# cmbant/getdist

Hardware: AMD Instinct MI355X
Metric: 2D KDE densities/sec (triangle, 50 params, 1e+07 samples) (higher is better)
Workload: dtype f64

## Files before the change

### getdist_amd/csrc/binning.hip

```cpp
#include "ctx.hpp"

#include <array>
#include <map>

#define LDS_HIST_BYTES (128 * 1024)

struct BinDiv {
    double binmin, width, rcp;
};
__device__ __forceinline__ BinDiv make_bindiv(double binmin, double width) {
    BinDiv d;
    d.binmin = binmin, d.width = width;
    const unsigned long long mant = (unsigned long long)__double_as_longlong(width) & 0xFFFFFFFFFFFFFull;
    d.rcp = (mant == 0xFFFFFFFFFFFFFull) ? 0.0 : 1.0 / width;
    return d;
}
__device__ __forceinline__ double bin_quotient(double x, const BinDiv& d) {
    const double n = x - d.binmin;
    double q = n * d.rcp;
    double r = fma(-q, d.width, n);
    q = fma(r, d.rcp, q);
    r = fma(-q, d.width, n);
    q = fma(r, d.rcp, q);
    if (!(fabs(q) < 1e300) || d.rcp == 0.0) q = n / d.width;
// ... 201 lines not shown
            const uint4 ax = gload_u4(P.ix + i);
            const uint4 ay = gload_u4(P.iy + i);
            double2 wv[4];
#pragma unroll
            for (int q = 0; q < 4; ++q)
                wv[q] = HAS_W ? *reinterpret_cast<const double2*>(w + i + 2 * q) : make_double2(1.0, 1.0);
            const unsigned xs[4] = {ax.x, ax.y, ax.z, ax.w}, ys[4] = {ay.x, ay.y, ay.z, ay.w};
#pragma unroll
            for (int q = 0; q < 4; ++q) {
#pragma unroll
                for (int h = 0; h < 2; ++h) {
                    const unsigned cx = (xs[q] >> (16 * h)) & 0xFFFFu, cy = (ys[q] >> (16 * h)) & 0xFFFFu;
                    const unsigned r = cy - (unsigned)row0;
                    if (r < (unsigned)R && cx < (unsigned)F && cy < (unsigned)F)
                        lds_add<BinT>(&sh[r * F + cx], h ? wv[q].y : wv[q].x);
                }
            }
        }
        if (threadIdx.x == 0)
            for (int64_t i = hi8; i < hi; ++i) {
                const unsigned cx = P.ix[i], cy = P.iy[i];
                const unsigned r = cy - (unsigned)row0;
                if (r < (unsigned)R && cx < (unsigned)F && cy < (unsigned)F)
                    lds_add<BinT>(&sh[r * F + cx], HAS_W ? w[i] : 1.0);
            }
    } else {
        const int64_t hi2 = lo + ((hi - lo) & ~(int64_t)1);
        for (int64_t i = lo + 2 * (int64_t)threadIdx.x; i < hi2; i += 2 * (int64_t)blockDim.x) {
            const double2 xv = gload_d2(P.x + i);
            const double2 yv = gload_d2(P.y + i);
            double2 wv = make_double2(1.0, 1.0);
            if (HAS_W) wv = *reinterpret_cast<const double2*>(w + i);
            int cx0, cy0, cx1, cy1;
            if (MODE == 0) {
                cx0 = bin_round(xv.x, bdx), cy0 = bin_round(yv.x, bdy);
                cx1 = bin_round(xv.y, bdx), cy1 = bin_round(yv.y, bdy);
            } else {
                cx0 = bin_trunc(xv.x, bdx), cx1 = bin_trunc(xv.y, bdx);
                const double p0 = P.r0 * xv.x + P.r1 * yv.x, p1 = P.r0 * xv.y + P.r1 * yv.y;
                cy0 = bin_trunc(p0, bdy), cy1 = bin_trunc(p1, bdy);
            }
            unsigned r = (unsigned)cy0 - (unsigned)row0;
            if (r < (unsigned)R && (unsigned)cx0 < (unsigned)F && (unsigned)cy0 < (unsigned)F)
                lds_add<BinT>(&sh[r * F + cx0], wv.x);
            r = (unsigned)cy1 - (unsigned)row0;
            if (r < (unsigned)R && (unsigned)cx1 < (unsigned)F && (unsigned)cy1 < (unsigned)F)
                lds_add<BinT>(&sh[r * F + cx1], wv.y);
        }
        if (threadIdx.x == 0 && hi2 < hi) {
            const double xv = P.x[hi2], yv = P.y[hi2];
            int cx, cy;
            if (MODE == 0) {
                cx = bin_round(xv, bdx), cy = bin_round(yv, bdy);
            } else {
                cx = bin_trunc(xv, bdx);
                cy = bin_trunc(P.r0 * xv + P.r1 * yv, bdy);
            }
            const unsigned r = (unsigned)cy - (unsigned)row0;
            if (r < (unsigned)R && (unsigned)cx < (unsigned)F && (unsigned)cy < (unsigned)F)
                lds_add<BinT>(&sh[r * F + cx], HAS_W ? w[hi2] : 1.0);
        }
    }
    __syncthreads();
    flush_stripe<BinT>(sh, row0, R, F, hist_all + (int64_t)pair * F * F, nchunks == 1);
}


template <bool HAS_W8>
__global__ void __launch_bounds__(1024) k_hist2d_u16(const Hist2DPair* __restrict__ pairs, int B, int64_t N, int F,
                                                     int R, int nstripes, const unsigned char* __restrict__ w8,
                                                     double* __restrict__ hist_all, int* __restrict__ overflow) {
    extern __shared__ double sh_raw[];
    unsigned int* sh = reinterpret_cast<unsigned int*>(sh_raw);
    __shared__ double red[16];
    int pair, chunk, stripe;
    decode_block(nstripes, 1, pair, chunk, stripe);
    if (pair >= B) return;
    const Hist2DPair P = pairs[pair];
    const BinDiv bdx = make_bindiv(P.bx, P.wx), bdy = make_bindiv(P.by, P.wy);
    const int row0 = stripe * R;
    const int nwords = (R * F + 1) / 2;
    for (int i = threadIdx.x; i < nwords; i += blockDim.x) sh[i] = 0;
    __syncthreads();
    unsigned int nacc = 0;
    auto visit = [&](unsigned cx, unsigned cy, unsigned wt) {
        const unsigned r = cy - (unsigned)row0;
        if (r < (unsigned)R && cx < (unsigned)F && cy < (unsigned)F && (!HAS_W8 || wt != 0u)) {
            const unsigned a = r * (unsigned)F + cx;
            atomicAdd(&sh[a >> 1], wt << ((a & 1u) * 16u));
            nacc += wt;
        }
    };
    auto visit8 = [&](const uint4& ax, const uint4& ay, unsigned wlo, unsigned whi) {
        const unsigned xs[4] = {ax.x, ax.y, ax.z, ax.w}, ys[4] = {ay.x, ay.y, ay.z, ay.w};
#pragma unroll
        for (int q = 0; q < 4; ++q) {
            const unsigned ww = (q < 2 ? wlo : whi) >> ((q & 1) * 16);
            visit(xs[q] & 0xFFFFu, ys[q] & 0xFFFFu, HAS_W8 ? (ww & 0xFFu) : 1u);
            visit(xs[q] >> 16, ys[q] >> 16, HAS_W8 ? ((ww >> 8) & 0xFFu) : 1u);
        }
    };
    const int64_t N16 = N & ~(int64_t)15;
    for (int64_t i = 16 * (int64_t)threadIdx.x; i < N16; i += 16 * (int64_t)blockDim.x) {
        const uint4 ax0 = gload_u4(P.ix + i), ay0 = gload_u4(P.iy + i);
        const uint4 ax1 = gload_u4(P.ix + i + 8), ay1 = gload_u4(P.iy + i + 8);
        uint4 wv = make_uint4(0, 0, 0, 0);
        if (HAS_W8) wv = *reinterpret_cast<const uint4*>(w8 + i);
        visit8(ax0, ay0, wv.x, wv.y);
        visit8(ax1, ay1, wv.z, wv.w);
    }
    if (threadIdx.x == 0)
        for (int64_t i = N16; i < N; ++i) visit(P.ix[i], P.iy[i], HAS_W8 ? (unsigned)w8[i] : 1u);
    __syncthreads();
    double* hist = hist_all + (int64_t)pair * F * F;
    unsigned int total = 0;
    for (int i = threadIdx.x; i < R * F; i += blockDim.x) {
        const int r = row0 + i / F;
        if (r >= F) break;
        const unsigned int v = (sh[i >> 1] >> ((i & 1) * 16)) & 0xFFFFu;
        total += v;
        hist[(int64_t)r * F + (i % F)] = (double)v;
    }
    const double t = block_sum((double)total, red), a = block_sum((double)nacc, red);
    if (threadIdx.x == 0 && t != a) atomicOr(&overflow[pair], 1);
}

struct Hist2DPair8 {
    const unsigned char* ix;
    const unsigned char* iy;
};

template <int DEPTH>
__global__ void __launch_bounds__(1024) k_hist2d_u8_pf(const Hist2DPair8* __restrict__ pairs, int B, int64_t N,
                                                       double* __restrict__ hist_all, int* __restrict__ overflow, int nchunks = 1,
                                                       unsigned int* __restrict__ part = nullptr) {
    extern __shared__ double sh_raw[];
    unsigned int* sh = reinterpret_cast<unsigned int*>(sh_raw);
    double* red = sh_raw + 16384;
    const int units = B * nchunks, per_xcd = (units + 7) / 8;
    const int unit = (blockIdx.x & 7) * per_xcd + (blockIdx.x >> 3);
    if (unit >= units || (int)(blockIdx.x >> 3) >= per_xcd) return;
    const int pair = unit / nchunks, chunk = unit - pair * nchunks;
    const Hist2DPair8 P = pairs[pair];
    const int64_t nvec_all = N >> 4;
    int64_t per = (nvec_all + nchunks - 1) / nchunks;
    per = (per + 1023) & ~(int64_t)1023;
    const int64_t v0 = min(nvec_all, (int64_t)chunk * per), v1 = (nchunks == 1) ? nvec_all : min(nvec_all, v0 + per);
    const bool last = chunk == nchunks - 1;
    const uint4* gx = reinterpret_cast<const uint4*>(P.ix) + v0;
    const uint4* gy = reinterpret_cast<const uint4*>(P.iy) + v0;
    for (int i = threadIdx.x; i < 32768; i += 1024) sh[i] = 0;
    __syncthreads();
    auto visit2 = [&](unsigned v) {
        atomicAdd(&sh[v & 0x7fffu], __builtin_amdgcn_ubfe(v, 15, 1) * 0xffffu + 1u);
        atomicAdd(&sh[__builtin_amdgcn_ubfe(v, 16, 15)], (v >> 31) * 0xffffu + 1u);
    };
    auto visit16 = [&](const uint4& ax, const uint4& ay) {
        const unsigned xs[4] = {ax.x, ax.y, ax.z, ax.w}, ys[4] = {ay.x, ay.y, ay.z, ay.w};
#pragma unroll
        for (int q = 0; q < 4; ++q) {
            visit2(__builtin_amdgcn_perm(ys[q], xs[q], 0x05010400u));
            visit2(__builtin_amdgcn_perm(ys[q], xs[q], 0x07030602u));
        }
    };
    const int64_t nvec = v1 - v0;
    const int64_t K = (nvec >> 10) / DEPTH * DEPTH;
    if (K > 0) {
        uint4 rx[DEPTH], ry[DEPTH];
#pragma unroll
        for (int d = 0; d < DEPTH; ++d) {
            rx[d] = gload_u4(gx + d * 1024 + threadIdx.x), ry[d] = gload_u4(gy + d * 1024 + threadIdx.x);
            __builtin_amdgcn_sched_barrier(0);
        }
        for (int64_t k = 0; k < K; k += DEPTH) {
            const int64_t kn = (k + DEPTH < K ? k + DEPTH : K - DEPTH) * 1024 + threadIdx.x;
#pragma unroll
            for (int d = 0; d < DEPTH; ++d) {
                visit16(rx[d], ry[d]);
                rx[d] = gload_u4(gx + kn + d * 1024), ry[d] = gload_u4(gy + kn + d * 1024);
                __builtin_amdgcn_sched_barrier(0);
            }
        }
    }
    for (int64_t u = K * 1024 + threadIdx.x; u < nvec; u += 1024) visit16(gload_u4(gx + u), gload_u4(gy + u));
    if (threadIdx.x == 0 && last)
        for (int64_t i = nvec_all << 4; i < N; ++i) {
            const unsigned a = ((unsigned)P.iy[i] << 8) | (unsigned)P.ix[i];
            atomicAdd(&sh[a & 0x7fffu], (a >> 15) * 0xffffu + 1u);
        }
    __syncthreads();
    if (nchunks > 1) {
        unsigned int* out = part + (int64_t)unit * 32768;
        unsigned int total = 0;
        for (int i = 4 * threadIdx.x; i < 32768; i += 4096) {
            const uint4 c = *reinterpret_cast<const uint4*>(&sh[i]);
            total += (c.x & 0xffffu) + (c.x >> 16) + (c.y & 0xffffu) + (c.y >> 16) + (c.z & 0xffffu) + (c.z >> 16) + (c.w & 0xffffu) + (c.w >> 16);
            *reinterpret_cast<uint4*>(&out[i]) = c;
        }
        const double t = block_sum((double)total, red);
        const double mine = (double)((v1 - v0) << 4) + (last ? (double)(N - (nvec_all << 4)) : 0.0);
        if (threadIdx.x == 0 && t != mine) atomicOr(&overflow[pair], 1);
        return;
    }
    double* hist = hist_all + (int64_t)pair * 65536;
    unsigned int total = 0;
    for (int i = 2 * threadIdx.x; i < 32768; i += 2048) {
        const uint2 c = *reinterpret_cast<const uint2*>(&sh[i]);
        total += (c.x & 0xffffu) + (c.x >> 16) + (c.y & 0xffffu) + (c.y >> 16);
        *reinterpret_cast<double2*>(&hist[i]) = make_double2((double)(c.x & 0xffffu), (double)(c.y & 0xffffu));
        *reinterpret_cast<double2*>(&hist[i + 32768]) = make_double2((double)(c.x >> 16), (double)(c.y >> 16));
    }
    const double t = block_sum((double)total, red);
    if (threadIdx.x == 0 && t != (double)N) atomicOr(&overflow[pair], 1);
}

__global__ void __launch_bounds__(256) k_p8_reduce(const unsigned int* __restrict__ part, int nchunks, double* __restrict__ hist_all) {
    const int pair = blockIdx.y;
    const int i = (blockIdx.x * 256 + threadIdx.x) * 4;
    const unsigned int* p = part + (int64_t)pair * nchunks * 32768 + i;
    unsigned int lo[4] = {0, 0, 0, 0}, hi[4] = {0, 0, 0, 0};
    for (int c = 0; c < nchunks; ++c) {
        const uint4 v = *reinterpret_cast<const uint4*>(p + (int64_t)c * 32768);
        lo[0] += v.x & 0xffffu, hi[0] += v.x >> 16, lo[1] += v.y & 0xffffu, hi[1] += v.y >> 16;
        lo[2] += v.z & 0xffffu, hi[2] += v.z >> 16, lo[3] += v.w & 0xffffu, hi[3] += v.w >> 16;
    }
    double* hist = hist_all + (int64_t)pair * 65536;
    *reinterpret_cast<double2*>(&hist[i]) = make_double2((double)lo[0], (double)lo[1]);
    *reinterpret_cast<double2*>(&hist[i + 2]) = make_double2((double)lo[2], (double)lo[3]);
    *reinterpret_cast<double2*>(&hist[i + 32768]) = make_double2((double)hi[0], (double)hi[1]);
    *reinterpret_cast<double2*>(&hist[i + 32768 + 2]) = make_double2((double)hi[2], (double)hi[3]);
}

static int pick_chunks(const gd_ctx* ctx, int64_t units, int64_t rows);
static int u8_chunks(const gd_ctx* ctx, int B, int64_t N) {
    if (B >= 2 * ctx->cu_count) return 1;
    return pick_chunks(ctx, B, N);
}

struct PrebinCol8 {
    const double* x;
    unsigned char* idx;
    double binmin, width;
};

__global__ void __launch_bounds__(256) k_prebin8_batch(const PrebinCol8* __restrict__ colsv, int64_t N, int F,
                                                       unsigned long long* __restrict__ bad) {
    const PrebinCol8 C = colsv[blockIdx.y];
    const BinDiv bd = make_bindiv(C.binmin, C.width);
    const int64_t gtid = (int64_t)blockIdx.x * 256 + threadIdx.x, gsz = (int64_t)gridDim.x * 256;
    const int64_t N8 = N & ~(int64_t)7;
    unsigned nbad = 0;
    for (int64_t i = 8 * gtid; i < N8; i += 8 * gsz) {
        double2 v[4];
#pragma unroll
        for (int q = 0; q < 4; ++q) v[q] = gload_d2(C.x + i + 2 * q);
        unsigned o[8];
#pragma unroll
        for (int q = 0; q < 4; ++q) {
            const int a = bin_round(v[q].x, bd), b = bin_round(v[q].y, bd);
            nbad += ((unsigned)a >= (unsigned)F) + ((unsigned)b >= (unsigned)F);
            o[2 * q] = (unsigned)a & 0xffu;
            o[2 * q + 1] = (unsigned)b & 0xffu;
        }
        uint2 pk;
        pk.x = o[0] | (o[1] << 8) | (o[2] << 16) | (o[3] << 24);
        pk.y = o[4] | (o[5] << 8) | (o[6] << 16) | (o[7] << 24);
        *reinterpret_cast<uint2*>(C.idx + i) = pk;
    }
    if (gtid == 0)
        for (int64_t i = N8; i < N; ++i) {
            const int a = bin_round(C.x[i], bd);
            nbad += ((unsigned)a >= (unsigned)F);
            C.idx[i] = (unsigned char)a;
        }
    if (nbad) atomicAdd(&bad[blockIdx.y], (unsigned long long)nbad);
}

struct PrebinColB {
    const double* x;
    const unsigned short* bq;
    void* idx;
    double binmin, width;
    double mn, inv_scale, slack;
    int nb, pad;
};

__global__ void __launch_bounds__(256) k_bucket_lut(const PrebinColB* __restrict__ colsv, int F, int nbmax,
                                                    unsigned short* __restrict__ lut) {
    const PrebinColB C = colsv[blockIdx.y];
    const int b = blockIdx.x * 256 + threadIdx.x;
    if (b >= C.nb) return;
    unsigned short v = 0xFFFF;
    if (b > 0 && b < C.nb - 1) {
        const BinDiv bd = make_bindiv(C.binmin, C.width);
        const double x_lo = (C.mn + ((double)b - 1e-3) * C.inv_scale) - C.slack;
        const double x_hi = (C.mn + ((double)b + 1.0 + 1e-3) * C.inv_scale) + C.slack;
        const int a = bin_round(x_lo, bd), c = bin_round(x_hi, bd);
        if (a == c && (unsigned)a < (unsigned)F) v = (unsigned short)a;
    }
    lut[(int64_t)blockIdx.y * nbmax + b] = v;
}

template <bool OUT8>
__global__ void __launch_bounds__(512) k_prebin_bq(const PrebinColB* __restrict__ colsv, int64_t N, int64_t R, int cap, int nbmax,
                                                   const unsigned short* __restrict__ lut, unsigned int* __restrict__ lists,
                                                   int* __restrict__ counts) {
    extern __shared__ unsigned short slut[];
    __shared__ int nlist;
    const PrebinColB C = colsv[blockIdx.y];
    {
        const uint4* src = reinterpret_cast<const uint4*>(lut + (int64_t)blockIdx.y * nbmax);
        uint4* dst = reinterpret_cast<uint4*>(slut);
        for (int i = threadIdx.x; i < C.nb / 8; i += 512) dst[i] = src[i];
    }
    if (threadIdx.x == 0) nlist = 0;
    __syncthreads();
    const int mask = C.nb - 1;
    unsigned int* mylist = lists + ((int64_t)blockIdx.y * gridDim.x + blockIdx.x) * cap;
    const int64_t g_lo = (int64_t)blockIdx.x * R / 8;
    int64_t g_hi = g_lo + R / 8;
    if (g_hi > N / 8) g_hi = N / 8;
    auto group = [&](const uint4& v, int64_t g) {
        const unsigned wd[4] = {v.x, v.y, v.z, v.w};
        unsigned o[8];
#pragma unroll
        for (int e = 0; e < 8; ++e) {
            unsigned r = slut[(wd[e >> 1] >> (16 * (e & 1))) & mask];
            if (r == 0xFFFFu) {
                const int pos = atomicAdd(&nlist, 1);
                if (pos < cap) mylist[pos] = (unsigned)(8 * g + e);
                r = 0;
            }
            o[e] = r;
        }
        if (OUT8) {
            uint2 pk;
            pk.x = o[0] | (o[1] << 8) | (o[2] << 16) | (o[3] << 24);
            pk.y = o[4] | (o[5] << 8) | (o[6] << 16) | (o[7] << 24);
            *reinterpret_cast<uint2*>((unsigned char*)C.idx + 8 * g) = pk;
        } else {
            uint4 pk;
            pk.x = o[0] | (o[1] << 16), pk.y = o[2] | (o[3] << 16), pk.z = o[4] | (o[5] << 16), pk.w = o[6] | (o[7] << 16);
            *reinterpret_cast<uint4*>((unsigned short*)C.idx + 8 * g) = pk;
        }
    };
    constexpr int U = 4;
    int64_t i = g_lo + threadIdx.x;
    for (; i + (U - 1) * 512 < g_hi; i += U * 512) {
        uint4 v[U];
#pragma unroll
        for (int q = 0; q < U; ++q) v[q] = gload_u4(C.bq + 8 * (i + q * 512));
#pragma unroll
        for (int q = 0; q < U; ++q) group(v[q], i + q * 512);
    }
    for (; i < g_hi; i += 512) group(gload_u4(C.bq + 8 * i), i);
    __syncthreads();
    if (threadIdx.x == 0) counts[(int64_t)blockIdx.y * gridDim.x + blockIdx.x] = nlist;
}

template <bool OUT8>
__global__ void __launch_bounds__(256) k_prebin_fix(const PrebinColB* __restrict__ colsv, int64_t N, int64_t R, int cap, int F,
                                                    const unsigned int* __restrict__ lists, const int* __restrict__ counts,
                                                    unsigned long long* __restrict__ bad) {
    const PrebinColB C = colsv[blockIdx.y];
    const BinDiv bd = make_bindiv(C.binmin, C.width);
    unsigned nbad = 0;
    auto settle = [&](int64_t row) {
        const int a = bin_round(C.x[row], bd);
        if (OUT8) {
            nbad += ((unsigned)a >= (unsigned)F);
            ((unsigned char*)C.idx)[row] = (unsigned char)a;
        } else {
            ((unsigned short*)C.idx)[row] = (unsigned)a < (unsigned)F ? (unsigned short)a : (unsigned short)0xFFFF;
        }
    };
    const int cnt = counts[(int64_t)blockIdx.y * gridDim.x + blockIdx.x];
    if (cnt <= cap) {
        const unsigned int* mylist = lists + ((int64_t)blockIdx.y * gridDim.x + blockIdx.x) * cap;
        int k = threadIdx.x;
        for (; k + 3 * 256 < cnt; k += 4 * 256) {
            unsigned int r[4];
#pragma unroll
            for (int q = 0; q < 4; ++q) r[q] = mylist[k + q * 256];
            double xv[4];
#pragma unroll
            for (int q = 0; q < 4; ++q) xv[q] = C.x[r[q]];
#pragma unroll
            for (int q = 0; q < 4; ++q) {
                const int a = bin_round(xv[q], bd);
                if (OUT8) {
                    nbad += ((unsigned)a >= (unsigned)F);
                    ((unsigned char*)C.idx)[r[q]] = (unsigned char)a;
                } else {
                    ((unsigned short*)C.idx)[r[q]] = (unsigned)a < (unsigned)F ? (unsigned short)a : (unsigned short)0xFFFF;
                }
            }
        }
        for (; k < cnt; k += 256) settle((int64_t)mylist[k]);
    } else {
        const int64_t lo = (int64_t)blockIdx.x * R;
        int64_t hi = lo + R;
        if (hi > N / 8 * 8) hi = N / 8 * 8;
        for (int64_t r = lo + threadIdx.x; r < hi; r += 256) settle(r);
    }
    if (blockIdx.x == gridDim.x - 1)
        for (int64_t r = N / 8 * 8 + threadIdx.x; r < N; r += 256) settle(r);
    if (OUT8 && nbad) atomicAdd(&bad[blockIdx.y], (unsigned long long)nbad);
}

struct BucketRoute {
    std::vector<PrebinColB> recs;
    std::vector<int> slot_of;
    int nbmax = 0;
};
static BucketRoute bucket_route(gd_ctx* ctx, const int32_t* cols, int32_t ncols, const double* binmin, const double* width,
                                void* const* d_idx) {
    BucketRoute R;
    R.slot_of.assign((size_t)ncols, -1);
    if (!ctx->bq || getenv("GDHIP_NO_BUCKET_COLS")) return R;
    {
        const char* e = getenv("GDHIP_BUCKET_ROUTE_MIN");
        const int min_cols = e ? atoi(e) : 24;
        if (ncols < min_cols) return R;
    }
    BucketCols& B = *ctx->bq;
    std::lock_guard<std::mutex> g(B.mu);
    if (!B.buf || B.ld != ctx->ld) return R;
    for (int c = 0; c < ncols; ++c) {
        const int col = cols[c];
        if (col < 0 || col >= B.n || B.nb[col] <= 0) continue;
        PrebinColB r;
        memset(&r, 0, sizeof r);
        r.x = ctx->cols + (int64_t)col * ctx->ld;
        r.bq = B.buf + (int64_t)col * B.ld;
        r.idx = d_idx[c];
        r.binmin = binmin[c], r.width = width[c];
        r.mn = B.mn[col];
        r.inv_scale = 1.0 / B.scale[col];
        const double mx = r.mn + (double)B.nb[col] * r.inv_scale;
        r.slack = 8.0 * 2.220446049250313e-16 * fmax(fabs(r.mn), fabs(mx));
        r.nb = B.nb[col];
        if (!(r.inv_scale > 0) || !std::isfinite(r.inv_scale) || !std::isfinite(r.slack)) continue;
        R.slot_of[c] = (int)R.recs.size();
        R.recs.push_back(r);
        if (r.nb > R.nbmax) R.nbmax = r.nb;
    }
    return R;
}
struct BucketShape {
    int nblk;
    int64_t R;
    int cap;
};
static BucketShape bucket_shape(const gd_ctx* ctx, int nc) {
    BucketShape S;
    int nblk = (4 * ctx->cu_count + nc - 1) / nc;
    int64_t R = (ctx->N + nblk - 1) / nblk;
    if (R < 131072) R = 131072;
    R = (R + 4095) / 4096 * 4096;
    nblk = (int)((ctx->N + R - 1) / R);
    if (nblk < 1) nblk = 1;
    S.nblk = nblk, S.R = R, S.cap = (int)(R / 8);
    if (const char* e = getenv("GDHIP_BUCKET_LIST_CAP"))
        if (atoi(e) > 0 && atoi(e) < S.cap) S.cap = atoi(e);
    return S;
}
static int64_t bucket_route_bytes(const gd_ctx* ctx, const BucketRoute& R) {
    if (R.recs.empty()) return 0;
    const int nc = (int)R.recs.size();
    const BucketShape S = bucket_shape(ctx, nc);
    return ((int64_t)nc * sizeof(PrebinColB) + 255) / 256 * 256 + ((int64_t)nc * R.nbmax * 2 + 255) / 256 * 256 +
           ((int64_t)nc * 8 + 255) / 256 * 256 + ((int64_t)nc * S.nblk * 4 + 255) / 256 * 256 + (int64_t)nc * S.nblk * S.cap * 4 + 256;
}
template <bool OUT8>
static int bucket_route_launch(gd_ctx* ctx, const BucketRoute& R, char* base, int F, unsigned long long** bad_dev) {
    const int nc = (int)R.recs.size();
    const BucketShape S = bucket_shape(ctx, nc);
    int64_t off = 0;
    auto take = [&](int64_t bytes) {
        int64_t o = off;
        off += (bytes + 255) / 256 * 256;
        return o;
    };
    const int64_t o_recs = take((int64_t)nc * sizeof(PrebinColB)), o_lut = take((int64_t)nc * R.nbmax * 2), o_bad = take((int64_t)nc * 8),
                  o_cnt = take((int64_t)nc * S.nblk * 4), o_list = take((int64_t)nc * S.nblk * S.cap * 4);
    PrebinColB* d_recs = (PrebinColB*)(base + o_recs);
    unsigned short* d_lut = (unsigned short*)(base + o_lut);
    unsigned long long* d_bad = (unsigned long long*)(base + o_bad);
    int* d_cnt = (int*)(base + o_cnt);
    unsigned int* d_list = (unsigned int*)(base + o_list);
    GD_TRY(gd_h2d(ctx, d_recs, R.recs.data(), (size_t)nc * sizeof(PrebinColB)));
    GD_HIP(hipMemsetAsync(d_bad, 0, (size_t)nc * 8, ctx->stream));
    k_bucket_lut<<<dim3(R.nbmax / 256, nc), 256, 0, ctx->stream>>>(d_recs, F, R.nbmax, d_lut);
    GD_KERNEL_CHECK();
    const size_t lds = (size_t)R.nbmax * 2;
    GD_HIP(hipFuncSetAttribute((const void*)k_prebin_bq<OUT8>, hipFuncAttributeMaxDynamicSharedMemorySize, (int)lds));
    k_prebin_bq<OUT8><<<dim3(S.nblk, nc), 512, lds, ctx->stream>>>(d_recs, ctx->N, S.R, S.cap, R.nbmax, d_lut, d_list, d_cnt);
    GD_KERNEL_CHECK();
    k_prebin_fix<OUT8><<<dim3(S.nblk, nc), 256, 0, ctx->stream>>>(d_recs, ctx->N, S.R, S.cap, F, d_list, d_cnt, d_bad);
    GD_KERNEL_CHECK();
    *bad_dev = d_bad;
    return GD_OK;
}

#ifndef P16_UNROLL
#define P16_UNROLL 4
#endif
template <int MODE>
__global__ void __launch_bounds__(1024) k_hist2d_f64_p16(const Hist2DPair* __restrict__ pairs, int B, int64_t N, int F, int R,
                                                         int nstripes, int nchunks, int tile_major,
                                                         unsigned int* __restrict__ part, int* __restrict__ overflow) {
    extern __shared__ double sh_raw[];
    unsigned int* sh = reinterpret_cast<unsigned int*>(sh_raw);
    __shared__ double red[16];
    int pair, chunk, stripe;
    if (tile_major)
        decode_block_tiles(B, nstripes, nchunks, pair, chunk, stripe);
    else
        decode_block(nstripes, nchunks, pair, chunk, stripe);
    if (pair >= B) return;
    const Hist2DPair P = pairs[pair];
    const BinDiv bdx = make_bindiv(P.bx, P.wx), bdy = make_bindiv(P.by, P.wy);
    const int row0 = stripe * R;
    const int nwords = (R * F + 1) / 2;
    for (int i = threadIdx.x; i < nwords; i += 1024) sh[i] = 0;
    __syncthreads();
    int64_t per = (N + nchunks - 1) / nchunks;
    per = (per + 7) & ~(int64_t)7;
    const int64_t lo = (int64_t)chunk * per;
    int64_t hi = lo + per;
    if (hi > N) hi = N;
    if (hi < lo) hi = lo;
    unsigned int nacc = 0;
    auto visit = [&](double xv, double yv) {
        int cx, cy;
        if (MODE == 0) {
            cx = bin_round(xv, bdx), cy = bin_round(yv, bdy);
        } else {
            cx = bin_trunc(xv, bdx);
            cy = bin_trunc(P.r0 * xv + P.r1 * yv, bdy);
        }
        const unsigned r = (unsigned)cy - (unsigned)row0;
        if (r < (unsigned)R && (unsigned)cx < (unsigned)F && (unsigned)cy < (unsigned)F) {
            const unsigned a = r * (unsigned)F + (unsigned)cx;
            atomicAdd(&sh[a >> 1], 1u << ((a & 1u) * 16u));
            nacc += 1;
        }
    };
    const int64_t hi2 = lo + ((hi - lo) & ~(int64_t)1);
    int64_t i = lo + 2 * (int64_t)threadIdx.x;
    for (; i + (int64_t)(P16_UNROLL - 1) * 2 * 1024 < hi2; i += (int64_t)P16_UNROLL * 2 * 1024) {
        double2 xv[P16_UNROLL], yv[P16_UNROLL];
#pragma unroll
        for (int u = 0; u < P16_UNROLL; ++u) {
            xv[u] = gload_d2(P.x + i + (int64_t)u * 2 * 1024);
            yv[u] = gload_d2(P.y + i + (int64_t)u * 2 * 1024);
        }
#pragma unroll
        for (int u = 0; u < P16_UNROLL; ++u) {
            visit(xv[u].x, yv[u].x);
            visit(xv[u].y, yv[u].y);
        }
    }
    for (; i < hi2; i += 2 * 1024) {
        const double2 xv = gload_d2(P.x + i);
        const double2 yv = gload_d2(P.y + i);
        visit(xv.x, yv.x);
        visit(xv.y, yv.y);
    }
    if (threadIdx.x == 0 && hi2 < hi) visit(P.x[hi2], P.y[hi2]);
    __syncthreads();
    unsigned int* dst = part + (((int64_t)pair * nchunks + chunk) * nstripes + stripe) * (int64_t)nwords;
    unsigned int total = 0;
    for (int i = threadIdx.x; i < nwords; i += 1024) {
        const unsigned int v = sh[i];
        total += (v & 0xffffu) + (v >> 16);
        dst[i] = v;
    }
    const double t = block_sum((double)total, red), a = block_sum((double)nacc, red);
    if (threadIdx.x == 0 && t != a) atomicOr(&overflow[pair], 1);
}

__global__ void __launch_bounds__(1024) k_hist2d_u16_chunks(const Hist2DPair* __restrict__ pairs, int B, int64_t N, int F, int R,
                                                            int nstripes, int nchunks, unsigned int* __restrict__ part,
                                                            int* __restrict__ overflow) {
    extern __shared__ double sh_raw[];
    unsigned int* sh = reinterpret_cast<unsigned int*>(sh_raw);
    __shared__ double red[16];
    int pair, chunk, stripe;
    decode_block(nstripes, nchunks, pair, chunk, stripe);
    if (pair >= B) return;
    const Hist2DPair P = pairs[pair];
    const int row0 = stripe * R;
    const int nwords = (R * F + 1) / 2;
    for (int i = threadIdx.x; i < nwords; i += 1024) sh[i] = 0;
    __syncthreads();
    int64_t per = (N + nchunks - 1) / nchunks;
    per = (per + 7) & ~(int64_t)7;
    const int64_t lo = (int64_t)chunk * per;
    int64_t hi = lo + per;
    if (hi > N) hi = N;
    unsigned int nacc = 0;
    auto visit = [&](unsigned cx, unsigned cy) {
        const unsigned r = cy - (unsigned)row0;
        if (r < (unsigned)R && cx < (unsigned)F && cy < (unsigned)F) {
            const unsigned a = r * (unsigned)F + cx;
            atomicAdd(&sh[a >> 1], 1u << ((a & 1u) * 16u));
            nacc += 1;
        }
    };
    const int64_t hi8 = lo < hi ? lo + ((hi - lo) & ~(int64_t)7) : lo;
    auto visit8 = [&](const uint4& ax, const uint4& ay) {
        const unsigned xs[4] = {ax.x, ax.y, ax.z, ax.w}, ys[4] = {ay.x, ay.y, ay.z, ay.w};
#pragma unroll
        for (int q = 0; q < 4; ++q) {
            visit(xs[q] & 0xFFFFu, ys[q] & 0xFFFFu);
            visit(xs[q] >> 16, ys[q] >> 16);
        }
    };
    constexpr int DEPTH = 3;
    const int64_t nvec = (hi8 - lo) >> 3;
    const int64_t K = (nvec >> 10) / DEPTH * DEPTH;
    const uint4* gx = reinterpret_cast<const uint4*>(P.ix + lo);
    const uint4* gy = reinterpret_cast<const uint4*>(P.iy + lo);
    if (K > 0) {
        uint4 rx[DEPTH], ry[DEPTH];
#pragma unroll
        for (int d = 0; d < DEPTH; ++d) {
            rx[d] = gload_u4(gx + d * 1024 + threadIdx.x), ry[d] = gload_u4(gy + d * 1024 + threadIdx.x);
            __builtin_amdgcn_sched_barrier(0);
        }
        for (int64_t k = 0; k < K; k += DEPTH) {
            const int64_t kn = (k + DEPTH < K ? k + DEPTH : K - DEPTH) * 1024 + threadIdx.x;
#pragma unroll
            for (int d = 0; d < DEPTH; ++d) {
                visit8(rx[d], ry[d]);
                rx[d] = gload_u4(gx + kn + d * 1024), ry[d] = gload_u4(gy + kn + d * 1024);
                __builtin_amdgcn_sched_barrier(0);
            }
        }
    }
    for (int64_t u = K * 1024 + threadIdx.x; u < nvec; u += 1024) visit8(gload_u4(gx + u), gload_u4(gy + u));
    if (threadIdx.x == 0)
        for (int64_t i = hi8; i < hi; ++i) visit(P.ix[i], P.iy[i]);
    __syncthreads();
    unsigned int* dst = part + (((int64_t)pair * nchunks + chunk) * nstripes + stripe) * (int64_t)nwords;
    unsigned int total = 0;
    for (int i = threadIdx.x; i < nwords; i += 1024) {
        const unsigned int v = sh[i];
        total += (v & 0xffffu) + (v >> 16);
        dst[i] = v;
    }
    const double t = block_sum((double)total, red), a = block_sum((double)nacc, red);
    if (threadIdx.x == 0 && t != a) atomicOr(&overflow[pair], 1);
}

__global__ void __launch_bounds__(256) k_p16_reduce(const unsigned int* __restrict__ part, int F, int R, int nstripes, int nchunks,
                                                    double* __restrict__ hist_all) {
    const int pair = blockIdx.z, stripe = blockIdx.y;
    const int nwords = (R * F + 1) / 2;
    const int rows = min(R, F - stripe * R);
    const int wd = blockIdx.x * 256 + threadIdx.x;
    if (2 * wd >= rows * F) return;
    const int64_t step = (int64_t)nstripes * nwords;
    const unsigned int* p = part + ((int64_t)pair * nchunks * nstripes + stripe) * (int64_t)nwords + wd;
    unsigned int lo = 0, hi = 0;
    int c = 0;
    for (; c + 8 <= nchunks; c += 8) {
        unsigned int v[8];
#pragma unroll
        for (int q = 0; q < 8; ++q) v[q] = __builtin_nontemporal_load(p + (c + q) * step);
#pragma unroll
        for (int q = 0; q < 8; ++q) lo += v[q] & 0xffffu, hi += v[q] >> 16;
    }
    for (; c < nchunks; ++c) {
        const unsigned int v = p[c * step];
        lo += v & 0xffffu, hi += v >> 16;
    }
    double* hist = hist_all + (int64_t)pair * F * F + (int64_t)stripe * R * F;
    hist[2 * wd] = (double)lo;
    if (2 * wd + 1 < rows * F) hist[2 * wd + 1] = (double)hi;
}

__global__ void k_minmax_affine(const Hist2DPair* __restrict__ pairs, int64_t N, double* __restrict__ part) {
    __shared__ double red[16];
    const Hist2DPair P = pairs[blockIdx.y];
    double mn = INFINITY, mx = -INFINITY;
    const int64_t gtid = (int64_t)blockIdx.x * blockDim.x + threadIdx.x, gsz = (int64_t)gridDim.x * blockDim.x;
    const int64_t Ne = N & ~(int64_t)1;
    for (int64_t i = 2 * gtid; i < Ne; i += 2 * gsz) {
        const double2 xv = gload_d2(P.x + i);
        const double2 yv = gload_d2(P.y + i);
        const double p0 = P.r0 * xv.x + P.r1 * yv.x, p1 = P.r0 * xv.y + P.r1 * yv.y;
        mn = fmin(mn, fmin(p0, p1));
        mx = fmax(mx, fmax(p0, p1));
    }
    if (gtid == 0 && Ne < N) {
        const double p0 = P.r0 * P.x[Ne] + P.r1 * P.y[Ne];
        mn = fmin(mn, p0);
        mx = fmax(mx, p0);
    }
    const double r0 = block_min(mn, red), r1 = block_max(mx, red);
    if (threadIdx.x == 0) {
        double* p = part + ((int64_t)blockIdx.y * gridDim.x + blockIdx.x) * 2;
        p[0] = r0, p[1] = r1;
    }
}

#define MMG_COLS 8
#define MMG_PAIRS 16
struct MinmaxGroup {
    const double* col[MMG_COLS];
    double r0[MMG_PAIRS], r1[MMG_PAIRS];
    int a[MMG_PAIRS], b[MMG_PAIRS];
    int ncols, npairs;
};

__global__ void __launch_bounds__(256) k_minmax_affine_grouped(const MinmaxGroup* __restrict__ groups, int64_t N,
                                                               double* __restrict__ part) {
    __shared__ double2 slot[MMG_COLS][256];
    __shared__ double red[16];
    const MinmaxGroup& G = groups[blockIdx.y];
    const int ncols = G.ncols, npairs = G.npairs;
    double mn[MMG_PAIRS], mx[MMG_PAIRS];
#pragma unroll
    for (int p = 0; p < MMG_PAIRS; ++p) mn[p] = INFINITY, mx[p] = -INFINITY;
    const int64_t gtid = (int64_t)blockIdx.x * blockDim.x + threadIdx.x, gsz = (int64_t)gridDim.x * blockDim.x;
    const int64_t Ne = N & ~(int64_t)1;
    for (int64_t i = 2 * gtid; i < Ne; i += 2 * gsz) {
        double2 v[MMG_COLS];
#pragma unroll
        for (int c = 0; c < MMG_COLS; ++c) v[c] = gload_d2(G.col[min(c, ncols - 1)] + i);
        __builtin_amdgcn_sched_barrier(0);
#pragma unroll
        for (int c = 0; c < MMG_COLS; ++c) slot[c][threadIdx.x] = v[c];
#pragma unroll
        for (int p = 0; p < MMG_PAIRS; ++p)
            if (p < npairs) {
                const double2 xv = slot[G.a[p]][threadIdx.x], yv = slot[G.b[p]][threadIdx.x];
                const double p0 = G.r0[p] * xv.x + G.r1[p] * yv.x, p1 = G.r0[p] * xv.y + G.r1[p] * yv.y;
                mn[p] = fmin(mn[p], fmin(p0, p1));
                mx[p] = fmax(mx[p], fmax(p0, p1));
            }
    }
    if (gtid == 0 && Ne < N) {
#pragma unroll
        for (int p = 0; p < MMG_PAIRS; ++p)
            if (p < npairs) {
                const double p0 = G.r0[p] * G.col[G.a[p]][Ne] + G.r1[p] * G.col[G.b[p]][Ne];
                mn[p] = fmin(mn[p], p0);
                mx[p] = fmax(mx[p], p0);
            }
    }
    double* out = part + ((int64_t)blockIdx.y * gridDim.x + blockIdx.x) * MMG_PAIRS * 2;
#pragma unroll
    for (int p = 0; p < MMG_PAIRS; ++p)
        if (p < npairs) {
            const double r0 = block_min(mn[p], red), r1 = block_max(mx[p], red);
            if (threadIdx.x == 0) out[2 * p] = r0, out[2 * p + 1] = r1;
        }
}

static int pick_chunks(const gd_ctx* ctx, int64_t units, int64_t rows) {
    int best = 1;
    double best_cost = 1e30;
    for (int c = 1; c <= 16; ++c) {
        if ((int64_t)c * 65536 > rows && c > 1) break;
        const int64_t blocks = units * c;
        const double rounds = (double)((blocks + ctx->cu_count - 1) / ctx->cu_count);
        const double cost = rounds / c + 0.004 * c;
        if (cost < best_cost - 1e-12) best_cost = cost, best = c;
    }
    return best;
}

template <int MODE>
static int launch_hist2d(gd_ctx* ctx, int B, const std::vector<Hist2DPair>& hp, int F, double* d_hist, bool allow_p16 = true);

template <int MODE>
static int launch_hist2d_p16(gd_ctx* ctx, int B, const std::vector<Hist2DPair>& hp, int F, double* d_hist) {
    int R = LDS_HIST_BYTES / (F * 2);
    if (R > F) R = F;
    const int nstripes = (F + R - 1) / R;
    int nchunks = pick_chunks(ctx, (int64_t)B * nstripes, ctx->N);
    const int nwords = (R * F + 1) / 2;
    int tile_major = 0;
    if (B >= 16 && nstripes == 1 && ctx->N >= (1 << 20) && getenv("GDHIP_P16_TILE_MAJOR") != nullptr) {
        int64_t tiles = (ctx->N + 131071) / 131072;
        const int64_t cap = ((int64_t)3 << 30) / ((int64_t)B * nwords * 4);
        if (tiles > cap) tiles = cap;
        if (tiles > nchunks) nchunks = (int)tiles, tile_major = 1;
    }
    const int units = (B * nchunks + 7) / 8 * 8;
    const int64_t nblocks = (int64_t)units * nstripes;
    int64_t off = 0;
    auto take = [&](int64_t bytes) {
        int64_t o = off;
        off += (bytes + 255) / 256 * 256;
        return o;
    };
    const int64_t o_pairs = take((int64_t)B * sizeof(Hist2DPair)), o_flags = take((int64_t)B * 4),
                  o_part = take((int64_t)B * nchunks * nstripes * nwords * 4);
// ... 988 lines not shown
```

Before: 50080.

## Fuse bucket prebin fix-up pass into LUT kernel with batched list appends

Merges the separate fix-up kernel into the LUT prebin kernel, so each block settles its undecided rows right after a block barrier. That removes one kernel launch and the per-block counts array. Undecided samples are now gathered into a per-lane bitmask and appended with one LDS atomicAdd per unrolled iteration instead of one per sample. The load loop is software-pipelined to prefetch the next batch, the fix-up gathers use 8-way ILP across 512 threads, and the block count rounds down instead of up. The cost is a longer kernel with more register pressure, and the settle phase now runs inside the tail of each prebin block rather than as a separately scheduled grid.

```diff
diff --git a/getdist_amd/csrc/binning.hip b/getdist_amd/csrc/binning.hip
--- a/getdist_amd/csrc/binning.hip
+++ b/getdist_amd/csrc/binning.hip
@@ -527,9 +527,9 @@
 }
 
 template <bool OUT8>
-__global__ void __launch_bounds__(512) k_prebin_bq(const PrebinColB* __restrict__ colsv, int64_t N, int64_t R, int cap, int nbmax,
+__global__ void __launch_bounds__(512) k_prebin_bq(const PrebinColB* __restrict__ colsv, int64_t N, int64_t R, int cap, int nbmax, int F,
                                                    const unsigned short* __restrict__ lut, unsigned int* __restrict__ lists,
-                                                   int* __restrict__ counts) {
+                                                   unsigned long long* __restrict__ bad) {
     extern __shared__ unsigned short slut[];
     __shared__ int nlist;
     const PrebinColB C = colsv[blockIdx.y];
@@ -545,18 +545,15 @@
     const int64_t g_lo = (int64_t)blockIdx.x * R / 8;
     int64_t g_hi = g_lo + R / 8;
     if (g_hi > N / 8) g_hi = N / 8;
-    auto group = [&](const uint4& v, int64_t g) {
+    auto group = [&](const uint4& v, int64_t g) -> unsigned {
         const unsigned wd[4] = {v.x, v.y, v.z, v.w};
-        unsigned o[8];
+        unsigned o[8], open = 0;
 #pragma unroll
         for (int e = 0; e < 8; ++e) {
-            unsigned r = slut[(wd[e >> 1] >> (16 * (e & 1))) & mask];
-            if (r == 0xFFFFu) {
-                const int pos = atomicAdd(&nlist, 1);
-                if (pos < cap) mylist[pos] = (unsigned)(8 * g + e);
-                r = 0;
-            }
-            o[e] = r;
+            const unsigned r = slut[(wd[e >> 1] >> (16 * (e & 1))) & mask];
+            const bool undecided = r == 0xFFFFu;
+            open |= undecided ? 1u << e : 0u;
+            o[e] = undecided ? 0u : r;
         }
         if (OUT8) {
             uint2 pk;
@@ -568,30 +565,50 @@
             pk.x = o[0] | (o[1] << 16), pk.y = o[2] | (o[3] << 16), pk.z = o[4] | (o[5] << 16), pk.w = o[6] | (o[7] << 16);
             *reinterpret_cast<uint4*>((unsigned short*)C.idx + 8 * g) = pk;
         }
+        return open;
+    };
+    auto append = [&](unsigned open, int64_t g0) {
+        if (open == 0) return;
+        int pos = atomicAdd(&nlist, __popc(open));
+        while (open) {
+            const int b = __ffs((int)open) - 1;
+            open &= open - 1;
+            if (pos < cap) mylist[pos] = (unsigned)(8 * (g0 + (int64_t)(b >> 3) * 512) + (b & 7));
+            ++pos;
+        }
     };
     constexpr int U = 4;
+    static_assert(U * 8 <= 32, "one mask bit per sample of a lane's U groups");
     int64_t i = g_lo + threadIdx.x;
-    for (; i + (U - 1) * 512 < g_hi; i += U * 512) {
+    if (i + (U - 1) * 512 < g_hi) {
         uint4 v[U];
 #pragma unroll
         for (int q = 0; q < U; ++q) v[q] = gload_u4(C.bq + 8 * (i + q * 512));
-#pragma unroll
-        for (int q = 0; q < U; ++q) group(v[q], i + q * 512);
-    }
-    for (; i < g_hi; i += 512) group(gload_u4(C.bq + 8 * i), i);
-    __syncthreads();
-    if (threadIdx.x == 0) counts[(int64_t)blockIdx.y * gridDim.x + blockIdx.x] = nlist;
-}
-
-template <bool OUT8>
-__global__ void __launch_bounds__(256) k_prebin_fix(const PrebinColB* __restrict__ colsv, int64_t N, int64_t R, int cap, int F,
-                                                    const unsigned int* __restrict__ lists, const int* __restrict__ counts,
-                                                    unsigned long long* __restrict__ bad) {
-    const PrebinColB C = colsv[blockIdx.y];
+        for (;;) {
+            const int64_t in = i + U * 512;
+            const bool more = in + (U - 1) * 512 < g_hi;
+            uint4 nx[U];
+            if (more) {
+#pragma unroll
+                for (int q = 0; q < U; ++q) nx[q] = gload_u4(C.bq + 8 * (in + q * 512));
+            }
+            unsigned open = 0;
+#pragma unroll
+            for (int q = 0; q < U; ++q) open |= group(v[q], i + q * 512) << (8 * q);
+            append(open, i);
+            i = in;
+            if (!more) break;
+#pragma unroll
+            for (int q = 0; q < U; ++q) v[q] = nx[q];
+        }
+    }
+    for (; i < g_hi; i += 512) append(group(gload_u4(C.bq + 8 * i), i), i);
+    __syncthreads();
+    const int cnt = nlist;
     const BinDiv bd = make_bindiv(C.binmin, C.width);
     unsigned nbad = 0;
-    auto settle = [&](int64_t row) {
-        const int a = bin_round(C.x[row], bd);
+    auto settle = [&](int64_t row, double xv) {
+        const int a = bin_round(xv, bd);
         if (OUT8) {
             nbad += ((unsigned)a >= (unsigned)F);
             ((unsigned char*)C.idx)[row] = (unsigned char)a;
@@ -599,37 +616,27 @@
             ((unsigned short*)C.idx)[row] = (unsigned)a < (unsigned)F ? (unsigned short)a : (unsigned short)0xFFFF;
         }
     };
-    const int cnt = counts[(int64_t)blockIdx.y * gridDim.x + blockIdx.x];
     if (cnt <= cap) {
-        const unsigned int* mylist = lists + ((int64_t)blockIdx.y * gridDim.x + blockIdx.x) * cap;
-        int k = threadIdx.x;
-        for (; k + 3 * 256 < cnt; k += 4 * 256) {
-            unsigned int r[4];
-#pragma unroll
-            for (int q = 0; q < 4; ++q) r[q] = mylist[k + q * 256];
-            double xv[4];
-#pragma unroll
-            for (int q = 0; q < 4; ++q) xv[q] = C.x[r[q]];
-#pragma unroll
-            for (int q = 0; q < 4; ++q) {
-                const int a = bin_round(xv[q], bd);
-                if (OUT8) {
-                    nbad += ((unsigned)a >= (unsigned)F);
-                    ((unsigned char*)C.idx)[r[q]] = (unsigned char)a;
-                } else {
-                    ((unsigned short*)C.idx)[r[q]] = (unsigned)a < (unsigned)F ? (unsigned short)a : (unsigned short)0xFFFF;
-                }
-            }
-        }
-        for (; k < cnt; k += 256) settle((int64_t)mylist[k]);
+        constexpr int V = 8;
+        for (int k = threadIdx.x; k < cnt; k += V * 512) {
+            unsigned int r[V];
+#pragma unroll
+            for (int q = 0; q < V; ++q) r[q] = mylist[k + q * 512 < cnt ? k + q * 512 : cnt - 1];
+            double xv[V];
+#pragma unroll
+            for (int q = 0; q < V; ++q) xv[q] = C.x[r[q]];
+#pragma unroll
+            for (int q = 0; q < V; ++q)
+                if (k + q * 512 < cnt) settle((int64_t)r[q], xv[q]);
+        }
     } else {
         const int64_t lo = (int64_t)blockIdx.x * R;
         int64_t hi = lo + R;
         if (hi > N / 8 * 8) hi = N / 8 * 8;
-        for (int64_t r = lo + threadIdx.x; r < hi; r += 256) settle(r);
+        for (int64_t r = lo + threadIdx.x; r < hi; r += 512) settle(r, C.x[r]);
     }
     if (blockIdx.x == gridDim.x - 1)
-        for (int64_t r = N / 8 * 8 + threadIdx.x; r < N; r += 256) settle(r);
+        for (int64_t r = N / 8 * 8 + threadIdx.x; r < N; r += 512) settle(r, C.x[r]);
     if (OUT8 && nbad) atomicAdd(&bad[blockIdx.y], (unsigned long long)nbad);
 }
 
@@ -679,7 +686,8 @@
 };
 static BucketShape bucket_shape(const gd_ctx* ctx, int nc) {
     BucketShape S;
-    int nblk = (4 * ctx->cu_count + nc - 1) / nc;
+    int nblk = 4 * ctx->cu_count / nc;
+    if (nblk < 1) nblk = 1;
     int64_t R = (ctx->N + nblk - 1) / nblk;
     if (R < 131072) R = 131072;
     R = (R + 4095) / 4096 * 4096;
@@ -695,7 +703,7 @@
     const int nc = (int)R.recs.size();
     const BucketShape S = bucket_shape(ctx, nc);
     return ((int64_t)nc * sizeof(PrebinColB) + 255) / 256 * 256 + ((int64_t)nc * R.nbmax * 2 + 255) / 256 * 256 +
-           ((int64_t)nc * 8 + 255) / 256 * 256 + ((int64_t)nc * S.nblk * 4 + 255) / 256 * 256 + (int64_t)nc * S.nblk * S.cap * 4 + 256;
+           ((int64_t)nc * 8 + 255) / 256 * 256 + (int64_t)nc * S.nblk * S.cap * 4 + 256;
 }
 template <bool OUT8>
 static int bucket_route_launch(gd_ctx* ctx, const BucketRoute& R, char* base, int F, unsigned long long** bad_dev) {
@@ -708,11 +716,10 @@
         return o;
     };
     const int64_t o_recs = take((int64_t)nc * sizeof(PrebinColB)), o_lut = take((int64_t)nc * R.nbmax * 2), o_bad = take((int64_t)nc * 8),
-                  o_cnt = take((int64_t)nc * S.nblk * 4), o_list = take((int64_t)nc * S.nblk * S.cap * 4);
+                  o_list = take((int64_t)nc * S.nblk * S.cap * 4);
     PrebinColB* d_recs = (PrebinColB*)(base + o_recs);
     unsigned short* d_lut = (unsigned short*)(base + o_lut);
     unsigned long long* d_bad = (unsigned long long*)(base + o_bad);
-    int* d_cnt = (int*)(base + o_cnt);
     unsigned int* d_list = (unsigned int*)(base + o_list);
     GD_TRY(gd_h2d(ctx, d_recs, R.recs.data(), (size_t)nc * sizeof(PrebinColB)));
     GD_HIP(hipMemsetAsync(d_bad, 0, (size_t)nc * 8, ctx->stream));
@@ -720,9 +727,7 @@
     GD_KERNEL_CHECK();
     const size_t lds = (size_t)R.nbmax * 2;
     GD_HIP(hipFuncSetAttribute((const void*)k_prebin_bq<OUT8>, hipFuncAttributeMaxDynamicSharedMemorySize, (int)lds));
-    k_prebin_bq<OUT8><<<dim3(S.nblk, nc), 512, lds, ctx->stream>>>(d_recs, ctx->N, S.R, S.cap, R.nbmax, d_lut, d_list, d_cnt);
-    GD_KERNEL_CHECK();
-    k_prebin_fix<OUT8><<<dim3(S.nblk, nc), 256, 0, ctx->stream>>>(d_recs, ctx->N, S.R, S.cap, F, d_list, d_cnt, d_bad);
+    k_prebin_bq<OUT8><<<dim3(S.nblk, nc), 512, lds, ctx->stream>>>(d_recs, ctx->N, S.R, S.cap, R.nbmax, F, d_lut, d_list, d_bad);
     GD_KERNEL_CHECK();
     *bad_dev = d_bad;
     return GD_OK;
```

After: 50240, median of 6. About the same (+0.3%).
